# mrluin/TextualDegRemoval

Measured on AMD Instinct MI355X. Metric: train images/sec (512x512, bs=4/GPU), higher is better.
Workload: dtype f32 (3xbf16-split MFMA: 24-bit operand significands on the full fp32 exponent range, fp32 accumulate; unscaled gradients, no loss scale, no step-skip guard; tensors fp32 -- the MASA-encoder ResidualBlock activations / gradients as three bf16 planes whose sum IS the fp32 value, bit for bit)

## Files before the change

### textualdegremoval_amd/csrc/tdr_masa.hip

```cpp
#include "tdr_common.h"
#include "../../include/tdr.h"

namespace {

__device__ __forceinline__ int wrap_idx(int v, int n) { return v < 0 ? v + n : v; }

__global__ void lr_blocks_fwd_kernel(const float* __restrict__ feat, int C, int H, int W, int py, int px, int ky, int kx,
                                     long total, float* __restrict__ blk) {
    const int BH = ky + 2, BW = kx + 2;
    for (long i = blockIdx.x * (long)blockDim.x + threadIdx.x; i < total; i += (long)gridDim.x * blockDim.x) {
        const int u = (int)(i % BW); long r = i / BW;
        const int v = (int)(r % BH); r /= BH;
        const int c = (int)(r % C); r /= C;
        const int p = (int)(r % (py * px)); const long n = r / (py * px);
        const int by = p / px, bx = p % px;
        const int y = min(max(by * ky + v - 1, 0), H - 1), x = min(max(bx * kx + u - 1, 0), W - 1);
        blk[i] = feat[((n * C + c) * H + y) * W + x];
    }
}

__global__ void lr_blocks_bwd_kernel(const float* __restrict__ dblk, int C, int H, int W, int py, int px, int ky, int kx,
                                     long total, float* __restrict__ dfeat) {
    const int BH = ky + 2, BW = kx + 2, P = py * px;
    for (long i = blockIdx.x * (long)blockDim.x + threadIdx.x; i < total; i += (long)gridDim.x * blockDim.x) {
        const int x = (int)(i % W); long r = i / W;
        const int y = (int)(r % H); r /= H;
        const int c = (int)(r % C); const long n = r / C;
        float s = 0.f;
        for (int Y = (y == 0 ? 0 : y + 1); Y <= (y == H - 1 ? H + 1 : y + 1); ++Y) {
            for (int X = (x == 0 ? 0 : x + 1); X <= (x == W - 1 ? W + 1 : x + 1); ++X) {
                for (int by = max(0, (Y - 2) / ky - 1); by < py && by * ky <= Y; ++by) {
                    const int v = Y - by * ky;
                    if (v < 0 || v >= BH) continue;
                    for (int bx = max(0, (X - 2) / kx - 1); bx < px && bx * kx <= X; ++bx) {
                        const int u = X - bx * kx;
                        if (u < 0 || u >= BW) continue;
                        s += dblk[(((n * P + by * px + bx) * C + c) * BH + v) * BW + u];
                    }
                }
            }
        }
        dfeat[i] = s;
    }
}

__global__ __launch_bounds__(1024) void patch_inv_norm_kernel(const float* __restrict__ x, int C, int H, int W, int OH,
                                                             int OW, int dil, int step, int off, long npos,
                                                             float* __restrict__ inv) {
    __shared__ float red[16][64];
    const int lane = threadIdx.x & 63, sl = threadIdx.x >> 6;
    const long pos = blockIdx.x * 64L + lane;
    const bool live = pos < npos;
    const long pc = live ? pos : npos - 1;
    const int ox = (int)(pc % OW); const long r = pc / OW;
    const int oy = (int)(r % OH); const long b = r / OH;
    int offs[9];
#pragma unroll
    for (int k = 0; k < 9; ++k) {
        const int yy = oy * step + off + (k / 3) * dil, xx = ox * step + off + (k % 3) * dil;
        offs[k] = (yy >= 0 && yy < H && xx >= 0 && xx < W) ? yy * W + xx : -1;
    }
    float s = 0.f;
    const long HW = (long)H * W;
    for (int c = sl; c < C; c += 16) {
        const float* xc = x + (b * C + c) * HW;
#pragma unroll
        for (int k = 0; k < 9; ++k) {
            const float v = offs[k] >= 0 ? xc[offs[k]] : 0.f;
            s += v * v;
        }
    }
    red[sl][lane] = s;
    __syncthreads();
    if (sl == 0 && live) {
        float t = 0.f;
#pragma unroll
        for (int q = 0; q < 16; ++q) t += red[q][lane];
        inv[pos] = 1.0f / fmaxf(sqrtf(t), 1e-12f);
    }
}

__global__ __launch_bounds__(256) void patch_inv_norm_wave_kernel(const float* __restrict__ x, int C, int H, int W, int OH,
                                                                 int OW, int dil, int step, int off, long npos,
                                                                 float* __restrict__ inv) {
    const long pos = blockIdx.x * 4L + (threadIdx.x >> 6);
    if (pos >= npos) return;
    const int lane = threadIdx.x & 63;
    const int ox = (int)(pos % OW); long r = pos / OW;
    const int oy = (int)(r % OH); const long b = r / OH;
    float s = 0.f;
    for (int c = lane; c < C; c += 64) {
        const float* xc = x + (b * C + c) * (long)H * W;
#pragma unroll
        for (int k = 0; k < 9; ++k) {
            const int yy = oy * step + off + (k / 3) * dil, xx = ox * step + off + (k % 3) * dil;
            if (yy >= 0 && yy < H && xx >= 0 && xx < W) {
                const float v = xc[(long)yy * W + xx];
                s += v * v;
            }
        }
    }
    s = wave_sum(s);
    if (lane == 0) inv[pos] = 1.0f / fmaxf(sqrtf(s), 1e-12f);
}

__device__ __forceinline__ int box_start(int idx, int size, int diameter) {
    int lo = idx - diameter / 2 - 1, hi = idx + diameter / 2 + 1;
    if (lo < 0) { lo = 0; hi = diameter + 1; }
    if (hi > size - 1) { hi = size - 1; lo = hi - (diameter + 1); }
    return lo;
}

__global__ __launch_bounds__(256) void coarse_argmax_box_kernel(const float* __restrict__ dots,
                                                               const float* __restrict__ invq,
                                                               const float* __restrict__ invk, int ND, int N, int P,
                                                               int Hr, int Wr, int diameter, int* __restrict__ index,
                                                               int* __restrict__ y1, int* __restrict__ x1) {
    __shared__ float sv[256];
    __shared__ int si[256];
    const int np = blockIdx.x, n = np / P;
    const int R = Hr * Wr;
    float best = -INFINITY; int bi = 0x7fffffff;
    for (int r = threadIdx.x; r < R; r += 256) {
        float s = 0.f;
        for (int d = 0; d < ND; ++d)
            s += dots[((long)d * N * P + np) * R + r] * invq[(long)d * N * P + np] * invk[((long)d * N + n) * R + r];
        if (s > best) { best = s; bi = r; }
    }
    sv[threadIdx.x] = best; si[threadIdx.x] = bi;
    __syncthreads();
    for (int o = 128; o > 0; o >>= 1) {
        if (threadIdx.x < o) {
            const float v2 = sv[threadIdx.x + o]; const int i2 = si[threadIdx.x + o];
            if (v2 > sv[threadIdx.x] || (v2 == sv[threadIdx.x] && i2 < si[threadIdx.x])) { sv[threadIdx.x] = v2; si[threadIdx.x] = i2; }
        }
        __syncthreads();
    }
    if (threadIdx.x == 0) {
        const int idx = si[0];
        index[np] = idx;
        x1[np] = box_start(idx % Wr, Wr, diameter);
        y1[np] = box_start(idx / Wr, Hr, diameter);
    }
}

__global__ void gather_ref_block_kernel(const float* __restrict__ feat, int C, int H, int W, const int* __restrict__ y1,
                                        const int* __restrict__ x1, int P, int side, int s, long total,
                                        float* __restrict__ out) {
    const int SS = side * s;
    for (long i = blockIdx.x * (long)blockDim.x + threadIdx.x; i < total; i += (long)gridDim.x * blockDim.x) {
        const int u = (int)(i % SS); long r = i / SS;
        const int v = (int)(r % SS); r /= SS;
        const int c = (int)(r % C); const long b = r / C;
        const long n = b / P;
        const int y = wrap_idx(y1[b] * s + v, H), x = wrap_idx(x1[b] * s + u, W);
        out[i] = feat[((n * C + c) * H + y) * W + x];
    }
}

__global__ void scatter_ref_block_kernel(const float* __restrict__ dblk, int C, int H, int W, const int* __restrict__ y1,
                                         const int* __restrict__ x1, int P, int side, long total,
                                         float* __restrict__ dfeat) {
    for (long i = blockIdx.x * (long)blockDim.x + threadIdx.x; i < total; i += (long)gridDim.x * blockDim.x) {
        const int x = (int)(i % W); long r = i / W;
        const int y = (int)(r % H); r /= H;
        const int c = (int)(r % C); const long n = r / C;
        float acc = 0.f;
        for (int p = 0; p < P; ++p) {
            const long b = n * P + p;
            const int by = y1[b], bx = x1[b];
#pragma unroll
            for (int wy = 0; wy < 2; ++wy) {
                const int v = y - wy * H - by;
                if (v < 0 || v >= side || (wy == 1) != (by + v < 0)) continue;
#pragma unroll
                for (int wx = 0; wx < 2; ++wx) {
                    const int u = x - wx * W - bx;
                    if (u < 0 || u >= side || (wx == 1) != (bx + u < 0)) continue;
                    acc += dblk[((b * C + c) * side + v) * side + u];
                }
            }
        }
        dfeat[i] += acc;
    }
}

__global__ __launch_bounds__(256) void fine_argmax_kernel(const float* __restrict__ dots, const float* __restrict__ invq,
                                                         const float* __restrict__ invk, long rows, int P, int R,
                                                         int* __restrict__ index_all, float* __restrict__ soft_att) {
    const long row = blockIdx.x * 4L + (threadIdx.x >> 6);
    if (row >= rows) return;
    const int lane = threadIdx.x & 63;
    const long b = row / P;
    const float iq = invq[row];
    float best = -INFINITY; int bi = 0x7fffffff;
    for (int r = lane; r < R; r += 64) {
        const float v = dots[row * R + r] * iq * invk[b * R + r];
        if (v > best) { best = v; bi = r; }
    }
#pragma unroll
    for (int o = 32; o > 0; o >>= 1) {
        const float v2 = __shfl_xor(best, o, 64); const int i2 = __shfl_xor(bi, o, 64);
        if (v2 > best || (v2 == best && i2 < bi)) { best = v2; bi = i2; }
    }
    if (lane == 0) { index_all[row] = bi; soft_att[row] = best; }
}

__global__ __launch_bounds__(256) void fine_search_bwd_kernel(const float* __restrict__ datt,
                                                             const float* __restrict__ soft_att,
                                                             const int* __restrict__ index_all,
                                                             const float* __restrict__ lrb, const float* __restrict__ refb,
                                                             const float* __restrict__ invq, const float* __restrict__ invk,
                                                             int C, int K, int D, float* __restrict__ dlrb,
                                                             float* __restrict__ drefb) {
    extern __shared__ float sm[];
    const int b = blockIdx.y, c = blockIdx.x;
    const int P = K * K, BS = K + 2, R1 = D - 2;
    float* s_da = sm;
    float* s_at = s_da + P;
    float* s_iq = s_at + P;
    float* s_ik = s_iq + P;
    int* s_ix = reinterpret_cast<int*>(s_ik + P);
    float* s_q = reinterpret_cast<float*>(s_ix + P);
    float* s_k = s_q + BS * BS;
    int* s_ry = reinterpret_cast<int*>(s_k + D * D);
    int* s_rx = s_ry + P;
    int* s_qo = s_rx + P;
    for (int p = threadIdx.x; p < P; p += 256) {
        const int ix = index_all[(long)b * P + p];
        s_da[p] = datt[(long)b * P + p];
        s_at[p] = soft_att[(long)b * P + p];
        s_iq[p] = invq[(long)b * P + p];
        s_ik[p] = invk[(long)b * R1 * R1 + ix];
        s_ix[p] = ix;
        s_ry[p] = ix / R1;
        s_rx[p] = ix % R1;
        s_qo[p] = (p / K) * BS + (p % K);
    }
    for (int i = threadIdx.x; i < BS * BS; i += 256) s_q[i] = lrb[((long)b * C + c) * BS * BS + i];
    for (int i = threadIdx.x; i < D * D; i += 256) s_k[i] = refb[((long)b * C + c) * D * D + i];
    __syncthreads();
    for (int i = threadIdx.x; i < BS * BS; i += 256) {
        const int y = i / BS, x = i % BS;
        float s = 0.f;
#pragma unroll
        for (int k = 0; k < 9; ++k) {
            const int pyy = y - k / 3, pxx = x - k % 3;
            if (pyy < 0 || pyy >= K || pxx < 0 || pxx >= K) continue;
            const int p = pyy * K + pxx;
            const int ry = s_ry[p], rx = s_rx[p];
            const float kv = s_k[(ry + k / 3) * D + rx + k % 3];
            s += s_da[p] * s_iq[p] * (kv * s_ik[p] - s_at[p] * s_q[i] * s_iq[p]);
        }
        dlrb[((long)b * C + c) * BS * BS + i] = s;
    }
    for (int i = threadIdx.x; i < D * D; i += 256) {
        const int v = i / D, u = i % D;
        float s = 0.f;
        for (int p = 0; p < P; ++p) {
            const int kyy = v - s_ry[p], kxx = u - s_rx[p];
            if (kyy < 0 || kyy > 2 || kxx < 0 || kxx > 2) continue;
            const float qv = s_q[s_qo[p] + kyy * BS + kxx];
            s += s_da[p] * s_ik[p] * (qv * s_iq[p] - s_at[p] * s_k[i] * s_ik[p]);
        }
        drefb[((long)b * C + c) * D * D + i] = s;
    }
}

struct TrGeom {
    int src[9];
    float wgt;
    float inv_cnt;
    int a00, a01, a10, a11; float w00, w01, w10, w11;
};

__device__ __forceinline__ void tr_geometry(int Yl, int Xl, int b, const int* __restrict__ y1, const int* __restrict__ x1,
                                            const int* __restrict__ index_all, const float* __restrict__ soft_att, int K,
                                            int side, int s, int H, int W, TrGeom& g) {
    const int R1 = side - 2;
    const int i0 = Yl / s, j0 = Xl / s;
    int cnt = 0;
#pragma unroll
    for (int k = 0; k < 9; ++k) {
        const int i = i0 + k / 3 - 1, j = j0 + k % 3 - 1;
        g.src[k] = -1;
        if (i < 0 || i >= K || j < 0 || j >= K) continue;
        const int idx = index_all[(long)b * K * K + i * K + j];
        const int ry = idx / R1, rx = idx % R1;
        const int sy = ry * s + Yl - i * s + s, sx = rx * s + Xl - j * s + s;
        const int gy = wrap_idx(y1[b] * s + sy, H), gx = wrap_idx(x1[b] * s + sx, W);
        g.src[k] = gy * W + gx;
        ++cnt;
    }
    g.inv_cnt = 1.0f / (float)cnt;
    const float fy = fmaxf(((float)Yl + 0.5f) / (float)s - 0.5f, 0.f), fx = fmaxf(((float)Xl + 0.5f) / (float)s - 0.5f, 0.f);
    const int yy0 = min((int)fy, K - 1), xx0 = min((int)fx, K - 1);
    const int yy1 = min(yy0 + 1, K - 1), xx1 = min(xx0 + 1, K - 1);
    const float ly = fy - (float)yy0, lx = fx - (float)xx0;
    g.a00 = yy0 * K + xx0; g.a01 = yy0 * K + xx1; g.a10 = yy1 * K + xx0; g.a11 = yy1 * K + xx1;
    g.w00 = (1.f - ly) * (1.f - lx); g.w01 = (1.f - ly) * lx; g.w10 = ly * (1.f - lx); g.w11 = ly * lx;
    const float* at = soft_att + (long)b * K * K;
    const float top = at[g.a00] * (1.f - lx) + at[g.a01] * lx;
    const float bot = at[g.a10] * (1.f - lx) + at[g.a11] * lx;
    g.wgt = (top * (1.f - ly) + bot * ly);
}

constexpr int TR_CG = 8;

__global__ __launch_bounds__(256) void transfer_fwd_kernel(const float* __restrict__ feat, int C, int H, int W,
                                                          const int* __restrict__ y1, const int* __restrict__ x1,
                                                          const int* __restrict__ index_all,
                                                          const float* __restrict__ soft_att, int py, int px, int K,
                                                          int side, int s, float* __restrict__ out, long out_ns) {
    const int OW = px * K * s, OH = py * K * s;
    const int pix = blockIdx.x * 256 + threadIdx.x, n = blockIdx.z;
    if (pix >= OH * OW) return;
    const int Y = pix / OW, X = pix % OW;
    const int by = Y / (K * s), bx = X / (K * s);
    const int b = (n * py + by) * px + bx;
    TrGeom g;
    tr_geometry(Y - by * K * s, X - bx * K * s, b, y1, x1, index_all, soft_att, K, side, s, H, W, g);
    const long HWf = (long)H * W, HWo = (long)OH * OW;
    float mult[9];
#pragma unroll
    for (int k = 0; k < 9; ++k) {
        int m = 0;
        bool first = g.src[k] >= 0;
#pragma unroll
        for (int q = 0; q < 9; ++q) {
            const bool same = g.src[q] == g.src[k];
            m += same ? 1 : 0;
            if (q < k && same) first = false;
        }
        mult[k] = first ? (float)m : 0.f;
    }
    const int c0 = blockIdx.y * TR_CG;
    float accs[TR_CG];
#pragma unroll
    for (int i = 0; i < TR_CG; ++i) {
        const float* f = feat + ((long)n * C + min(c0 + i, C - 1)) * HWf;
        float acc = 0.f;
#pragma unroll
        for (int k = 0; k < 9; ++k)
            if (mult[k] != 0.f) acc += mult[k] * f[g.src[k]];
        accs[i] = acc;
    }
#pragma unroll
    for (int i = 0; i < TR_CG; ++i)
        if (c0 + i < C) out[(long)n * out_ns + (long)(c0 + i) * HWo + pix] = accs[i] * g.inv_cnt * g.wgt;
}

__global__ __launch_bounds__(256) void absmax_bits_kernel(const float* __restrict__ x, long x_ns, long per4, int N,
                                                         unsigned* __restrict__ out) {
    float m = 0.f;
    const f32x4* p = reinterpret_cast<const f32x4*>(x + (long)blockIdx.y * x_ns);
    for (long i = blockIdx.x * 256L + threadIdx.x; i < per4; i += (long)gridDim.x * 256) {
        const f32x4 v = p[i];
        m = fmaxf(fmaxf(m, fmaxf(fabsf(v[0]), fabsf(v[1]))), fmaxf(fabsf(v[2]), fabsf(v[3])));
    }
    m = wave_max(m);
    if ((threadIdx.x & 63) == 0) atomicMax(out, __float_as_uint(m));
}
__device__ __forceinline__ int fixed_shift(unsigned amax_bits) {
    const int e = (int)((amax_bits >> 23) & 0xff) - 127;
    return 46 - (e + 1);
}
__global__ void fixed_to_float_kernel(const long long* __restrict__ acc, long n, const unsigned* __restrict__ amax_bits,
                                      float* __restrict__ out) {
    const double inv = ldexp(1.0, -fixed_shift(amax_bits[0]));
    for (long i = blockIdx.x * 256L + threadIdx.x; i < n; i += (long)gridDim.x * 256) out[i] += (float)((double)acc[i] * inv);
}

template <bool FIXED>
__global__ __launch_bounds__(256) void transfer_bwd_kernel(const float* __restrict__ dout, long dout_ns,
                                                          const float* __restrict__ feat, int C, int H, int W,
                                                          const int* __restrict__ y1, const int* __restrict__ x1,
                                                          const int* __restrict__ index_all,
                                                          const float* __restrict__ soft_att, int py, int px, int K,
                                                          int side, int s, int cpb , int N,
                                                          const unsigned* __restrict__ amax_bits,
                                                          unsigned long long* __restrict__ dfacc ,
                                                          float* __restrict__ dfeat ,
                                                          float* __restrict__ dA ) {
    const int OW = px * K * s, OH = py * K * s;
    const int pix = blockIdx.x * 256 + threadIdx.x, n = blockIdx.z;
    if (pix >= OH * OW) return;
    const int Y = pix / OW, X = pix % OW;
    const int by = Y / (K * s), bx = X / (K * s);
    const int b = (n * py + by) * px + bx;
    TrGeom g;
    tr_geometry(Y - by * K * s, X - bx * K * s, b, y1, x1, index_all, soft_att, K, side, s, H, W, g);
    const long HWf = (long)H * W, HWo = (long)OH * OW;
    const float coef = g.inv_cnt * g.wgt;
    float mult[9];
#pragma unroll
    for (int k = 0; k < 9; ++k) {
        int m = 0;
        bool first = g.src[k] >= 0;
#pragma unroll
        for (int q = 0; q < 9; ++q) {
            const bool same = g.src[q] == g.src[k];
            m += same ? 1 : 0;
            if (q < k && same) first = false;
        }
        mult[k] = first ? (float)m : 0.f;
    }
    float da = 0.f;
    const int c0 = blockIdx.y * cpb, c1 = min(c0 + cpb, C);
    const int shift = FIXED ? fixed_shift(amax_bits[0]) : 0;
    const bool scatter = !FIXED || amax_bits[0] != 0u;
    for (int c = c0; c < c1; ++c) {
        const float* f = feat + ((long)n * C + c) * HWf;
        const float go = dout[(long)n * dout_ns + (long)c * HWo + pix];
        float acc = 0.f;
        const float gv = go * coef;
#pragma unroll
        for (int k = 0; k < 9; ++k)
            if (mult[k] > 0.f) {
                acc += mult[k] * f[g.src[k]];
                if (!scatter) continue;
                if (FIXED) atomicAdd(&dfacc[((long)n * C + c) * HWf + g.src[k]], (unsigned long long)__float2ll_rn(ldexpf(gv * mult[k], shift)));
                else atomicAdd(&dfeat[((long)n * C + c) * HWf + g.src[k]], gv * mult[k]);
            }
        da += go * acc * g.inv_cnt;
    }
    dA[((long)blockIdx.y * N + n) * HWo + pix] = da;
}

__global__ __launch_bounds__(64) void transfer_datt_kernel(const float* __restrict__ dA, int py, int px, int K, int s,
                                                          int chunks, long chunk_stride, float* __restrict__ datt) {
    const int b = blockIdx.x, e = blockIdx.y;
    const int P = py * px, n = b / P, by = (b % P) / px, bx = b % px;
    const int i = e / K, j = e % K;
    const int OW = px * K * s, OH = py * K * s, KS = K * s;
    const int ylo = max((i - 1) * s, 0), yhi = min((i + 2) * s, KS);
    const int xlo = max((j - 1) * s, 0), xhi = min((j + 2) * s, KS);
    const int nw = xhi - xlo, tot = (yhi - ylo) * nw;
    float acc = 0.f;
    for (int t = threadIdx.x; t < tot; t += 64) {
        const int Yl = ylo + t / nw, Xl = xlo + t % nw;
        const float fy = fmaxf(((float)Yl + 0.5f) / (float)s - 0.5f, 0.f), fx = fmaxf(((float)Xl + 0.5f) / (float)s - 0.5f, 0.f);
        const int yy0 = min((int)fy, K - 1), xx0 = min((int)fx, K - 1);
        const int yy1 = min(yy0 + 1, K - 1), xx1 = min(xx0 + 1, K - 1);
        const float ly = fy - (float)yy0, lx = fx - (float)xx0;
        float wgt = 0.f;
        if (yy0 == i && xx0 == j) wgt += (1.f - ly) * (1.f - lx);
        if (yy0 == i && xx1 == j) wgt += (1.f - ly) * lx;
        if (yy1 == i && xx0 == j) wgt += ly * (1.f - lx);
        if (yy1 == i && xx1 == j) wgt += ly * lx;
        if (wgt != 0.f) {
            const long o = (long)n * OH * OW + (long)(by * KS + Yl) * OW + bx * KS + Xl;
            float v = 0.f;
            for (int q = 0; q < chunks; ++q) v += dA[q * chunk_stride + o];
            acc += wgt * v;
        }
    }
    acc = wave_sum(acc);
    if (threadIdx.x == 0) datt[(long)b * K * K + e] += acc;
}

inline int grid1d(long total, int cap = 8192) {
    long b = (total + 255) / 256;
    return (int)(b < cap ? (b < 1 ? 1 : b) : cap);
}

}

extern "C" int tdr_lr_blocks_fwd(const float* feat, int N, int C, int H, int W, int py, int px, int ky, int kx, float* blk,
                                 void* stream) {
    TDR_REQUIRE(feat && blk, "tdr_lr_blocks_fwd: null pointer");
    const long total = (long)N * py * px * C * (ky + 2) * (kx + 2);
    hipLaunchKernelGGL(lr_blocks_fwd_kernel, dim3(grid1d(total)), dim3(256), 0, (hipStream_t)stream, feat, C, H, W, py, px, ky,
                       kx, total, blk);
    TDR_LAUNCH_CHECK("lr_blocks_fwd");
    return TDR_OK;
}

extern "C" int tdr_lr_blocks_bwd(const float* dblk, int N, int C, int H, int W, int py, int px, int ky, int kx,
                                 float* dfeat, void* stream) {
    TDR_REQUIRE(dblk && dfeat, "tdr_lr_blocks_bwd: null pointer");
    const long total = (long)N * C * H * W;
    hipLaunchKernelGGL(lr_blocks_bwd_kernel, dim3(grid1d(total)), dim3(256), 0, (hipStream_t)stream, dblk, C, H, W, py, px, ky,
                       kx, total, dfeat);
    TDR_LAUNCH_CHECK("lr_blocks_bwd");
    return TDR_OK;
}

extern "C" int tdr_patch_inv_norm(const float* x, int B, int C, int H, int W, int OH, int OW, int dil, int pad, int step,
                                  int off, float* inv, void* stream) {
    TDR_REQUIRE(x && inv, "tdr_patch_inv_norm: null pointer");
    const long npos = (long)B * OH * OW;
    if (npos >= 1024)
        hipLaunchKernelGGL(patch_inv_norm_kernel, dim3((unsigned)((npos + 63) / 64)), dim3(1024), 0, (hipStream_t)stream, x, C, H,
                           W, OH, OW, dil, step, off - pad, npos, inv);
    else
        hipLaunchKernelGGL(patch_inv_norm_wave_kernel, dim3((unsigned)((npos + 3) / 4)), dim3(256), 0, (hipStream_t)stream, x, C,
                           H, W, OH, OW, dil, step, off - pad, npos, inv);
    TDR_LAUNCH_CHECK("patch_inv_norm");
    return TDR_OK;
}

extern "C" int tdr_coarse_argmax_box(const float* dots, const float* invq, const float* invk, int ND, int N, int P, int Hr,
                                     int Wr, int diameter, int* index, int* y1, int* x1, void* stream) {
    TDR_REQUIRE(dots && invq && invk && index && y1 && x1, "tdr_coarse_argmax_box: null pointer");
    hipLaunchKernelGGL(coarse_argmax_box_kernel, dim3(N * P), dim3(256), 0, (hipStream_t)stream, dots, invq, invk, ND, N, P, Hr,
                       Wr, diameter, index, y1, x1);
    TDR_LAUNCH_CHECK("coarse_argmax_box");
    return TDR_OK;
}

extern "C" int tdr_gather_ref_block(const float* feat, int N, int C, int H, int W, const int* y1, const int* x1, int P,
                                    int side, int s, float* out, void* stream) {
    TDR_REQUIRE(feat && y1 && x1 && out, "tdr_gather_ref_block: null pointer");
    const long total = (long)N * P * C * side * s * side * s;
    hipLaunchKernelGGL(gather_ref_block_kernel, dim3(grid1d(total)), dim3(256), 0, (hipStream_t)stream, feat, C, H, W, y1, x1,
                       P, side, s, total, out);
    TDR_LAUNCH_CHECK("gather_ref_block");
    return TDR_OK;
}

extern "C" int tdr_scatter_ref_block(const float* dblk, int N, int C, int H, int W, const int* y1, const int* x1, int P,
                                     int side, float* dfeat, void* stream) {
    TDR_REQUIRE(dblk && y1 && x1 && dfeat, "tdr_scatter_ref_block: null pointer");
    const long total = (long)N * C * H * W;
    hipLaunchKernelGGL(scatter_ref_block_kernel, dim3(grid1d(total)), dim3(256), 0, (hipStream_t)stream, dblk, C, H, W, y1, x1,
                       P, side, total, dfeat);
    TDR_LAUNCH_CHECK("scatter_ref_block");
    return TDR_OK;
}

extern "C" int tdr_fine_argmax(const float* dots, const float* invq, const float* invk, int B, int P, int R, int* index_all,
                               float* soft_att, void* stream) {
    TDR_REQUIRE(dots && invq && invk && index_all && soft_att, "tdr_fine_argmax: null pointer");
    const long rows = (long)B * P;
    hipLaunchKernelGGL(fine_argmax_kernel, dim3((unsigned)((rows + 3) / 4)), dim3(256), 0, (hipStream_t)stream, dots, invq, invk,
                       rows, P, R, index_all, soft_att);
    TDR_LAUNCH_CHECK("fine_argmax");
    return TDR_OK;
}

extern "C" int tdr_fine_search_bwd(const float* datt, const float* soft_att, const int* index_all, const float* lrb,
                                   const float* refb, const float* invq, const float* invk, int B, int C, int K, int D,
                                   float* dlrb, float* drefb, void* stream) {
    TDR_REQUIRE(datt && soft_att && index_all && lrb && refb && invq && invk && dlrb && drefb, "tdr_fine_search_bwd: null pointer");
    const size_t lds = (size_t)(8 * K * K + (K + 2) * (K + 2) + D * D) * sizeof(float);
    hipLaunchKernelGGL(fine_search_bwd_kernel, dim3(C, B), dim3(256), lds, (hipStream_t)stream, datt, soft_att, index_all, lrb,
                       refb, invq, invk, C, K, D, dlrb, drefb);
    TDR_LAUNCH_CHECK("fine_search_bwd");
    return TDR_OK;
}

extern "C" int tdr_transfer_fwd(const float* feat, int N, int C, int H, int W, const int* y1, const int* x1,
                                const int* index_all, const float* soft_att, int py, int px, int K, int side, int s,
                                float* out, int64_t out_ns, void* stream) {
    TDR_REQUIRE(feat && y1 && x1 && index_all && soft_att && out, "tdr_transfer_fwd: null pointer");
    const long opix = (long)py * K * s * px * K * s;
    hipLaunchKernelGGL(transfer_fwd_kernel, dim3((unsigned)((opix + 255) / 256), tdr_cdiv(C, TR_CG), N), dim3(256), 0,
                       (hipStream_t)stream, feat, C, H, W, y1, x1, index_all, soft_att, py, px, K, side, s, out, (long)out_ns);
    TDR_LAUNCH_CHECK("transfer_fwd");
    return TDR_OK;
}

static int tdr_transfer_chunks(int N, int C, int py, int px, int K, int s) {
    const long opix = (long)py * K * s * px * K * s;
    const long pix_blocks = ((opix + 255) / 256) * N;
    long chunks = (1024 + pix_blocks - 1) / pix_blocks;
    if (chunks > C / 8) chunks = C / 8;
    if (chunks < 1) chunks = 1;
    return (int)chunks;
}

extern "C" int64_t tdr_transfer_ws_floats(int N, int C, int H, int W, int py, int px, int K, int s) {
    const int64_t opix = (int64_t)py * K * s * px * K * s;
    return (int64_t)tdr_transfer_chunks(N, C, py, px, K, s) * N * opix + 4 + 2 * (int64_t)N * C * H * W;
}

extern "C" int tdr_transfer_bwd(const float* dout, int64_t dout_ns, const float* feat, int N, int C, int H, int W,
                                const int* y1, const int* x1, const int* index_all, const float* soft_att, int py, int px,
                                int K, int side, int s, int deterministic, float* dfeat, float* datt, float* ws, void* stream) {
    TDR_REQUIRE(dout && feat && y1 && x1 && index_all && soft_att && dfeat && datt && ws, "tdr_transfer_bwd: null pointer");
    const long opix = (long)py * K * s * px * K * s;
    hipStream_t st = (hipStream_t)stream;
    const int chunks = tdr_transfer_chunks(N, C, py, px, K, s);
    const int cpb = tdr_cdiv(C, chunks);
    float* dA = ws;
    const dim3 grid((unsigned)((opix + 255) / 256), tdr_cdiv(C, cpb), N);
    if (!deterministic) {
        hipLaunchKernelGGL(transfer_bwd_kernel<false>, grid, dim3(256), 0, st, dout, (long)dout_ns, feat, C, H, W, y1, x1, index_all,
                           soft_att, py, px, K, side, s, cpb, N, (const unsigned*)nullptr, (unsigned long long*)nullptr, dfeat, dA);
    } else {
        TDR_REQUIRE(opix % 4 == 0 && dout_ns % 4 == 0 && (reinterpret_cast<uintptr_t>(dout) & 15) == 0, "tdr_transfer_bwd: dout must be 16-byte aligned");
        char* tail = reinterpret_cast<char*>(ws + (long)chunks * N * opix);
        tail += (8 - reinterpret_cast<uintptr_t>(tail) % 8) % 8;
        unsigned* amax = reinterpret_cast<unsigned*>(tail);
        unsigned long long* acc = reinterpret_cast<unsigned long long*>(tail + 8);
        const long nacc = (long)N * C * H * W;
        if (hipMemsetAsync(tail, 0, 8 + (size_t)nacc * 8, st) != hipSuccess) {
            tdr_set_error("tdr_transfer_bwd: hipMemsetAsync failed");
            return TDR_ERR_HIP;
        }
        const long per4 = (long)C * opix / 4;
        hipLaunchKernelGGL(absmax_bits_kernel, dim3(grid1d(per4, 512), N), dim3(256), 0, st, dout, (long)dout_ns, per4, N, amax);
        hipLaunchKernelGGL(transfer_bwd_kernel<true>, grid, dim3(256), 0, st, dout, (long)dout_ns, feat, C, H, W, y1, x1, index_all,
                           soft_att, py, px, K, side, s, cpb, N, amax, acc, (float*)nullptr, dA);
        hipLaunchKernelGGL(fixed_to_float_kernel, dim3(grid1d(nacc, 4096)), dim3(256), 0, st, reinterpret_cast<const long long*>(acc),
                           nacc, amax, dfeat);
    }
    hipLaunchKernelGGL(transfer_datt_kernel, dim3(N * py * px, K * K), dim3(64), 0, st, ws, py, px, K, s, tdr_cdiv(C, cpb),
                       (long)N * opix, datt);
    TDR_LAUNCH_CHECK("transfer_bwd");
    return TDR_OK;
}

__global__ __launch_bounds__(256) void absmax_bits_any_kernel(const float* __restrict__ x, long x_ns, long per, unsigned* __restrict__ slot) {
    const float* p = x + (long)blockIdx.y * x_ns;
    float m = 0.f;
    unsigned bad = 0;
    for (long i = blockIdx.x * 256L + threadIdx.x; i < per; i += (long)gridDim.x * 256) {
        const float v = fabsf(p[i]);
        if (!(v <= 3.4028235e38f)) bad = 0x7fc00000u;
        m = fmaxf(m, v);
    }
    unsigned b = __float_as_uint(m) | bad;
#pragma unroll
    for (int o = 32; o > 0; o >>= 1) b = max(b, (unsigned)__shfl_xor((int)b, o, 64));
    if ((threadIdx.x & 63) == 0) atomicMax(slot, b);
}

extern "C" int tdr_absmax_bits(const float* x, int64_t x_ns, int N, int64_t per, unsigned* slot, void* stream) {
    TDR_REQUIRE(x && slot && N > 0 && per > 0, "tdr_absmax_bits: bad argument");
    hipLaunchKernelGGL(absmax_bits_any_kernel, dim3(grid1d(per, 256), N), dim3(256), 0, (hipStream_t)stream, x, (long)x_ns, (long)per, slot);
    TDR_LAUNCH_CHECK("absmax_bits");
    return TDR_OK;
}
```

Measured before the change: 62.79.

## Batch channels per block in MASA backward kernels and unroll datt gather

fine_search_bwd now handles eight channels per block and reuses the per-patch geometry and attention scalars across them. transfer_bwd processes channels in groups of eight, so all loads for a group are issued before the scatter atomics, using 32-bit byte offsets and a launch-bounds occupancy hint. transfer_datt unrolls its chunk-sum gather four ways. These target the latency-bound MASA backward kernels. The costs are more LDS and registers per block, and fewer blocks for fine_search.

```diff
diff --git a/profiles/masa_bwd/ab_kernels.py b/profiles/masa_bwd/ab_kernels.py
--- /dev/null
+++ b/profiles/masa_bwd/ab_kernels.py
@@ -0,0 +1,158 @@
+import argparse
+import hashlib
+import json
+import os
+import shutil
+import subprocess
+import sys
+import tempfile
+
+ROOT = os.path.dirname(os.path.dirname(os.path.dirname(os.path.abspath(__file__))))
+N, PY, PX, KK, SIDE, HD = 4, 4, 4, 8, 15, 32
+LEVELS = [(16, 32), (8, 64), (4, 128), (2, 256), (1, 512)]
+PATTERNS = ('coherent', 'random')
+FINE = (64, 512, 8, 15)
+
+
+def digest(t):
+    return hashlib.sha256(t.detach().cpu().contiguous().numpy().tobytes()).hexdigest()[:16]
+
+
+def index_pattern(kind, B, K, R1, g):
+    import torch
+    if kind == 'random':
+        return torch.randint(0, R1 * R1, (B, K * K), generator=g)
+    r0 = torch.randint(0, R1 - K + 1, (B, 1, 1), generator=g)
+    c0 = torch.randint(0, R1 - K + 1, (B, 1, 1), generator=g)
+    return ((r0 + torch.arange(K).view(1, K, 1)) * R1 + c0 + torch.arange(K).view(1, 1, K)).reshape(B, K * K)
+
+
+def transfer_inputs(s, C, pattern):
+    import torch
+    g = torch.Generator().manual_seed(1000 * s + C + (7 if pattern == 'random' else 0))
+    B = N * PY * PX
+    return dict(feat=torch.randn(N, C, HD * s, HD * s, generator=g).cuda(),
+                dout=torch.randn(N, C, PY * KK * s, PX * KK * s, generator=g).cuda(),
+                y1=torch.randint(0, HD - SIDE + 1, (B,), generator=g).int().cuda(),
+                x1=torch.randint(0, HD - SIDE + 1, (B,), generator=g).int().cuda(),
+                index_all=index_pattern(pattern, B, KK, SIDE - 2, g).int().cuda(),
+                soft_att=(torch.rand(B, KK * KK, generator=g) * 0.8 + 0.2).cuda())
+
+
+def graph_time(fn):
+    import torch
+    fn()
+    torch.cuda.synchronize()
+    st = torch.cuda.Stream()
+    with torch.cuda.stream(st):
+        fn()
+        gr = torch.cuda.CUDAGraph()
+        with torch.cuda.graph(gr, stream=st):
+            for _ in range(20):
+                fn()
+    torch.cuda.synchronize()
+    gr.replay()
+    torch.cuda.synchronize()
+    ts = []
+    for _ in range(15):
+        a, b = torch.cuda.Event(enable_timing=True), torch.cuda.Event(enable_timing=True)
+        a.record()
+        gr.replay()
+        b.record()
+        torch.cuda.synchronize()
+        ts.append(a.elapsed_time(b) * 1000.0 / 20)
+    return sorted(ts)[len(ts) // 2]
+
+
+def child(tag, folder):
+    import torch
+    sys.path.insert(0, ROOT)
+    from textualdegremoval_amd import kernels as K
+    out = dict(lib=os.environ.get('TDR_LIB_PATH', 'default'), bits={}, us={})
+    for s, C in LEVELS:
+        for pattern in PATTERNS:
+            inp = transfer_inputs(s, C, pattern)
+            key = f's={s} C={C} {pattern}'
+
+            def run(det, dfeat, datt):
+                K.DETERMINISTIC = det
+                K.transfer_bwd(inp['dout'], inp['feat'], inp['y1'], inp['x1'], inp['index_all'], inp['soft_att'], PY, PX, KK, SIDE, s, dfeat, datt)
+
+            B = N * PY * PX
+            rec = {}
+            for det in (True, False):
+                for rep in range(1 if det else 2):
+                    dfeat, datt = torch.zeros_like(inp['feat']), torch.zeros(B, KK * KK, device='cuda')
+                    run(det, dfeat, datt)
+                    torch.cuda.synchronize()
+                    if det:
+                        rec['det dfeat'], rec['det datt'] = digest(dfeat), digest(datt)
+                    else:
+                        rec['float datt'] = digest(datt)
+                        if tag == 'parent' or rep == 0:
+                            torch.save(dfeat.cpu(), os.path.join(folder, f'{tag} {key} float{rep}.pt'))
+            out['bits'][key] = rec
+            dfeat, datt = torch.zeros_like(inp['feat']), torch.zeros(B, KK * KK, device='cuda')
+            for det in (False, True):
+                out['us'][f'{key} {"fixed" if det else "float"}'] = graph_time(lambda: run(det, dfeat, datt))
+            del inp, dfeat, datt
+    B, C, Kk, D = FINE
+    for pattern in PATTERNS:
+        g = torch.Generator().manual_seed(99 + (7 if pattern == 'random' else 0))
+        lrb, refb = torch.randn(B, C, Kk + 2, Kk + 2, generator=g).cuda(), torch.randn(B, C, D, D, generator=g).cuda()
+        datt, att = torch.randn(B, Kk * Kk, generator=g).cuda(), torch.rand(B, Kk * Kk, generator=g).cuda()
+        invq, invk = (torch.rand(B, Kk * Kk, generator=g) + 0.5).cuda(), (torch.rand(B, (D - 2) ** 2, generator=g) + 0.5).cuda()
+        ia = index_pattern(pattern, B, Kk, D - 2, g).int().cuda()
+        dl, dr = K.fine_search_bwd(datt, att, ia, lrb, refb, invq, invk, Kk, D)
+        torch.cuda.synchronize()
+        key = f'fine B={B} C={C} {pattern}'
+        out['bits'][key] = {'dlrb': digest(dl), 'drefb': digest(dr)}
+        out['us'][key] = graph_time(lambda: K.fine_search_bwd(datt, att, ia, lrb, refb, invq, invk, Kk, D))
+    with open(os.path.join(folder, tag + '.json'), 'w') as f:
+        json.dump(out, f)
+
+
+def main():
+    ap = argparse.ArgumentParser()
+    ap.add_argument('--parent')
+    ap.add_argument('--result', default=os.path.join(ROOT, 'textualdegremoval_amd', 'libtdr_hip.so'))
+    ap.add_argument('--child')
+    ap.add_argument('--dir')
+    a = ap.parse_args()
+    if a.child:
+        return child(a.child, a.dir)
+    import torch
+    folder = tempfile.mkdtemp(prefix='masa_bwd_ab_')
+    try:
+        for tag, lib in (('parent', a.parent), ('result', a.result)):
+            env = dict(os.environ, TDR_LIB_PATH=os.path.abspath(lib))
+            subprocess.run([sys.executable, os.path.abspath(__file__), '--child', tag, '--dir', folder], env=env, check=True, timeout=400)
+        P, R = (json.load(open(os.path.join(folder, t + '.json'))) for t in ('parent', 'result'))
+        print(f'parent {P["lib"]}\nresult {R["lib"]}\n')
+        print('## Bit identity, parent library against result (sha256 of the tensor bytes)\n')
+        print('| case | output | parent | result | |\n|---|---|---|---|---|')
+        bad = 0
+        for key, rec in P['bits'].items():
+            for name, h in rec.items():
+                same = R['bits'][key][name] == h
+                bad += not same
+                print(f'| {key} | {name} | {h} | {R["bits"][key][name]} | {"equal" if same else "DIFFERENT"} |')
+        print(f'\n{bad} outputs differ.\n')
+        print('## Float-atomic dfeat: max |a - b| / max |a|, two runs of the parent beside parent against result\n')
+        print('| case | max abs dfeat | parent run 0 vs run 1 | parent run 0 vs result run 0 |\n|---|---|---|---|')
+        for s, C in LEVELS:
+            for pattern in PATTERNS:
+                key = f's={s} C={C} {pattern}'
+                p0, p1, r0 = (torch.load(os.path.join(folder, f'{t} {key} float{i}.pt')).double() for t, i in (('parent', 0), ('parent', 1), ('result', 0)))
+                m = p0.abs().max().item()
+                print(f'| {key} | {m:.3e} | {(p0 - p1).abs().max().item() / m:.3e} | {(p0 - r0).abs().max().item() / m:.3e} |')
+        print('\n## Time per launch, microseconds (graph of 20, median of 15 replays)\n')
+        print('| launch | parent | result | result / parent |\n|---|---|---|---|')
+        for key, t in P['us'].items():
+            print(f'| {key} | {t:.1f} | {R["us"][key]:.1f} | {R["us"][key] / t:.2f} |')
+    finally:
+        shutil.rmtree(folder, ignore_errors=True)
+
+
+if __name__ == '__main__':
+    main()
diff --git a/profiles/masa_bwd/masa_rows.py b/profiles/masa_bwd/masa_rows.py
--- /dev/null
+++ b/profiles/masa_bwd/masa_rows.py
@@ -0,0 +1,58 @@
+import bisect
+import re
+import sqlite3
+import sys
+
+MASA = ('transfer_bwd_kernel', 'fine_search_bwd_kernel', 'transfer_datt_kernel')
+
+
+def short(n):
+    n = re.sub(r'\(anonymous namespace\)::', '', n)
+    return re.sub(r'\(.*', '', re.sub(r'^void ', '', n))
+
+
+def main():
+    c = sqlite3.connect(sys.argv[1])
+    rows = list(c.execute('select name, start, end, grid_x/workgroup_x, grid_y, grid_z, vgpr_count, lds_size from kernels '
+                          'where name not like "%spin_kernel%" order by start'))
+    steps = sum('fine_search_bwd_kernel' in r[0] for r in rows)
+    tot = sum(r[2] - r[1] for r in rows)
+    print(f'total kernel time {tot / 1e6 / steps:.2f} ms/step over {steps} steps; {len(rows) / steps:.0f} launches/step')
+    ev = sorted([(r[1], 1) for r in rows] + [(r[2], -1) for r in rows])
+    t, n, run = [], [], 0
+    for at, d in ev:
+        run += d
+        t.append(at)
+        n.append(run)
+    busy = sum(t[i + 1] - t[i] for i in range(len(t) - 1) if n[i] >= 1)
+    both = sum(t[i + 1] - t[i] for i in range(len(t) - 1) if n[i] >= 2)
+    print(f'some kernel running {busy / 1e6 / steps:.2f} ms/step, two or more running {both / 1e6 / steps:.2f} ms/step')
+
+    def shared(a, b):
+        s, i = 0, bisect.bisect_right(t, a) - 1
+        while i < len(t) - 1 and t[i] < b:
+            if n[i] >= 2:
+                s += min(t[i + 1], b) - max(t[i], a)
+            i += 1
+        return s
+
+    by_name, by_grid = {}, {}
+    for name, a, b, gx, gy, gz, vg, lds in rows:
+        k = short(name)
+        if not any(m in k for m in MASA):
+            continue
+        for d, key in ((by_name, k), (by_grid, (k, gx, gy, gz, vg, lds))):
+            e = d.setdefault(key, [0, 0, 0])
+            e[0] += 1
+            e[1] += b - a
+            e[2] += shared(a, b)
+    print('--- MASA backward kernels (the last column: share of their time with another kernel running)')
+    for k, (cnt, dur, sh) in sorted(by_name.items(), key=lambda x: -x[1][1]):
+        print(f'{dur / 1e6 / steps:8.3f} ms/step  n/step {cnt / steps:4.1f}  {k:32s} {100 * sh / dur:5.1f} %')
+    print('--- by grid (workgroups x,y,z)')
+    for (k, gx, gy, gz, vg, lds), (cnt, dur, sh) in sorted(by_grid.items(), key=lambda x: (x[0][0], -x[0][1])):
+        print(f'{dur / cnt / 1e3:8.1f} us  n/step {cnt / steps:4.1f}  grid({gx},{gy},{gz}) vgpr {vg} lds {lds}  {k:32s} {100 * sh / dur:5.1f} %')
+
+
+if __name__ == '__main__':
+    main()
diff --git a/textualdegremoval_amd/csrc/tdr_masa.hip b/textualdegremoval_amd/csrc/tdr_masa.hip
--- a/textualdegremoval_amd/csrc/tdr_masa.hip
+++ b/textualdegremoval_amd/csrc/tdr_masa.hip
@@ -206,6 +206,8 @@
     if (lane == 0) { index_all[row] = bi; soft_att[row] = best; }
 }
 
+constexpr int FS_FC = 8;
+
 __global__ __launch_bounds__(256) void fine_search_bwd_kernel(const float* __restrict__ datt,
                                                              const float* __restrict__ soft_att,
                                                              const int* __restrict__ index_all,
@@ -214,16 +216,16 @@
                                                              int C, int K, int D, float* __restrict__ dlrb,
                                                              float* __restrict__ drefb) {
     extern __shared__ float sm[];
-    const int b = blockIdx.y, c = blockIdx.x;
-    const int P = K * K, BS = K + 2, R1 = D - 2;
+    const int b = blockIdx.y, cg = blockIdx.x * FS_FC, nc = min(FS_FC, C - cg);
+    const int P = K * K, BS = K + 2, R1 = D - 2, BB = BS * BS, DD = D * D;
     float* s_da = sm;
     float* s_at = s_da + P;
     float* s_iq = s_at + P;
     float* s_ik = s_iq + P;
     int* s_ix = reinterpret_cast<int*>(s_ik + P);
     float* s_q = reinterpret_cast<float*>(s_ix + P);
-    float* s_k = s_q + BS * BS;
-    int* s_ry = reinterpret_cast<int*>(s_k + D * D);
+    float* s_k = s_q + FS_FC * BB;
+    int* s_ry = reinterpret_cast<int*>(s_k + FS_FC * DD);
     int* s_rx = s_ry + P;
     int* s_qo = s_rx + P;
     for (int p = threadIdx.x; p < P; p += 256) {
@@ -237,33 +239,50 @@
         s_rx[p] = ix % R1;
         s_qo[p] = (p / K) * BS + (p % K);
     }
-    for (int i = threadIdx.x; i < BS * BS; i += 256) s_q[i] = lrb[((long)b * C + c) * BS * BS + i];
-    for (int i = threadIdx.x; i < D * D; i += 256) s_k[i] = refb[((long)b * C + c) * D * D + i];
+    for (int i = threadIdx.x; i < FS_FC * BB; i += 256) s_q[i] = i < nc * BB ? lrb[((long)b * C + cg) * BB + i] : 0.f;
+    for (int i = threadIdx.x; i < FS_FC * DD; i += 256) s_k[i] = i < nc * DD ? refb[((long)b * C + cg) * DD + i] : 0.f;
     __syncthreads();
-    for (int i = threadIdx.x; i < BS * BS; i += 256) {
+    for (int i = threadIdx.x; i < BB; i += 256) {
         const int y = i / BS, x = i % BS;
-        float s = 0.f;
+        float s[FS_FC];
+#pragma unroll
+        for (int j = 0; j < FS_FC; ++j) s[j] = 0.f;
 #pragma unroll
         for (int k = 0; k < 9; ++k) {
             const int pyy = y - k / 3, pxx = x - k % 3;
             if (pyy < 0 || pyy >= K || pxx < 0 || pxx >= K) continue;
             const int p = pyy * K + pxx;
-            const int ry = s_ry[p], rx = s_rx[p];
-            const float kv = s_k[(ry + k / 3) * D + rx + k % 3];
-            s += s_da[p] * s_iq[p] * (kv * s_ik[p] - s_at[p] * s_q[i] * s_iq[p]);
-        }
-        dlrb[((long)b * C + c) * BS * BS + i] = s;
-    }
-    for (int i = threadIdx.x; i < D * D; i += 256) {
+            const int ko = (s_ry[p] + k / 3) * D + s_rx[p] + k % 3;
+            const float da = s_da[p], at = s_at[p], iq = s_iq[p], ik = s_ik[p];
+#pragma unroll
+            for (int j = 0; j < FS_FC; ++j) {
+                const float kv = s_k[j * DD + ko];
+                s[j] += da * iq * (kv * ik - at * s_q[j * BB + i] * iq);
+            }
+        }
+#pragma unroll
+        for (int j = 0; j < FS_FC; ++j)
+            if (j < nc) dlrb[((long)b * C + cg + j) * BB + i] = s[j];
+    }
+    for (int i = threadIdx.x; i < DD; i += 256) {
         const int v = i / D, u = i % D;
-        float s = 0.f;
+        float s[FS_FC], kc[FS_FC];
+#pragma unroll
+        for (int j = 0; j < FS_FC; ++j) { s[j] = 0.f; kc[j] = s_k[j * DD + i]; }
         for (int p = 0; p < P; ++p) {
             const int kyy = v - s_ry[p], kxx = u - s_rx[p];
             if (kyy < 0 || kyy > 2 || kxx < 0 || kxx > 2) continue;
-            const float qv = s_q[s_qo[p] + kyy * BS + kxx];
-            s += s_da[p] * s_ik[p] * (qv * s_iq[p] - s_at[p] * s_k[i] * s_ik[p]);
-        }
-        drefb[((long)b * C + c) * D * D + i] = s;
+            const int qo = s_qo[p] + kyy * BS + kxx;
+            const float da = s_da[p], at = s_at[p], iq = s_iq[p], ik = s_ik[p];
+#pragma unroll
+            for (int j = 0; j < FS_FC; ++j) {
+                const float qv = s_q[j * BB + qo];
+                s[j] += da * ik * (qv * iq - at * kc[j] * ik);
+            }
+        }
+#pragma unroll
+        for (int j = 0; j < FS_FC; ++j)
+            if (j < nc) drefb[((long)b * C + cg + j) * DD + i] = s[j];
     }
 }
 
@@ -371,17 +390,71 @@
     for (long i = blockIdx.x * 256L + threadIdx.x; i < n; i += (long)gridDim.x * 256) out[i] += (float)((double)acc[i] * inv);
 }
 
+#ifndef TDR_TRB_CG
+#define TDR_TRB_CG 8
+#endif
+constexpr int TRB_CG = TDR_TRB_CG;
+
+template <bool FIXED, bool FULL>
+__device__ __forceinline__ void transfer_bwd_group(const float* __restrict__ dout_n , unsigned& po , long HWo,
+                                                   const float* __restrict__ feat, long HWf, long nC, int cb, int nv,
+                                                   unsigned (&so)[9] , const float (&mult)[9], float coef, float inv_cnt,
+                                                   bool scatter, int shift, unsigned long long* __restrict__ dfacc,
+                                                   float* __restrict__ dfeat, float& da) {
+    const char* fp = reinterpret_cast<const char*>(feat + (nC + cb) * HWf);
+    const char* op = reinterpret_cast<const char*>(dout_n + (long)cb * HWo);
+    char* dp = FIXED ? reinterpret_cast<char*>(dfacc + (nC + cb) * HWf) : reinterpret_cast<char*>(dfeat + (nC + cb) * HWf);
+    asm volatile("" : "+v"(po));
+    float go[TRB_CG], fv[TRB_CG][9];
+#pragma unroll
+    for (int k = 0; k < 9; ++k) asm volatile("" : "+v"(so[k]));
+#pragma unroll
+    for (int i = 0; i < TRB_CG; ++i) {
+        const int j = FULL ? i : min(i, nv - 1);
+        go[i] = *reinterpret_cast<const float*>(op + j * HWo * 4 + po);
+    }
+#pragma unroll
+    for (int k = 0; k < 9; ++k)
+        if (mult[k] > 0.f) {
+#pragma unroll
+            for (int i = 0; i < TRB_CG; ++i) {
+                const int j = FULL ? i : min(i, nv - 1);
+                fv[i][k] = *reinterpret_cast<const float*>(fp + j * HWf * 4 + so[k]);
+            }
+        }
+#pragma unroll
+    for (int i = 0; i < TRB_CG; ++i) {
+        float acc = 0.f;
+#pragma unroll
+        for (int k = 0; k < 9; ++k)
+            if (mult[k] > 0.f) acc += mult[k] * fv[i][k];
+        if (FULL || i < nv) da += go[i] * acc * inv_cnt;
+    }
+    if (!scatter) return;
+#pragma unroll
+    for (int k = 0; k < 9; ++k)
+        if (mult[k] > 0.f) {
+#pragma unroll
+            for (int i = 0; i < TRB_CG; ++i) {
+                if (!FULL && i >= nv) continue;
+                const float gv = go[i] * coef;
+                if (FIXED) atomicAdd(reinterpret_cast<unsigned long long*>(dp + i * HWf * 8 + so[k] * 2u), (unsigned long long)__float2ll_rn(ldexpf(gv * mult[k], shift)));
+                else atomicAdd(reinterpret_cast<float*>(dp + i * HWf * 4 + so[k]), gv * mult[k]);
+            }
+        }
+}
+
 template <bool FIXED>
-__global__ __launch_bounds__(256) void transfer_bwd_kernel(const float* __restrict__ dout, long dout_ns,
-                                                          const float* __restrict__ feat, int C, int H, int W,
-                                                          const int* __restrict__ y1, const int* __restrict__ x1,
-                                                          const int* __restrict__ index_all,
-                                                          const float* __restrict__ soft_att, int py, int px, int K,
-                                                          int side, int s, int cpb , int N,
-                                                          const unsigned* __restrict__ amax_bits,
-                                                          unsigned long long* __restrict__ dfacc ,
-                                                          float* __restrict__ dfeat ,
-                                                          float* __restrict__ dA ) {
+__global__ __launch_bounds__(256, 4) void transfer_bwd_kernel(const float* __restrict__ dout, long dout_ns,
+                                                             const float* __restrict__ feat, int C, int H, int W,
+                                                             const int* __restrict__ y1, const int* __restrict__ x1,
+                                                             const int* __restrict__ index_all,
+                                                             const float* __restrict__ soft_att, int py, int px, int K,
+                                                             int side, int s, int cpb , int N,
+                                                             const unsigned* __restrict__ amax_bits,
+                                                             unsigned long long* __restrict__ dfacc ,
+                                                             float* __restrict__ dfeat ,
+                                                             float* __restrict__ dA ) {
     const int OW = px * K * s, OH = py * K * s;
     const int pix = blockIdx.x * 256 + threadIdx.x, n = blockIdx.z;
     if (pix >= OH * OW) return;
@@ -409,23 +482,21 @@
     const int c0 = blockIdx.y * cpb, c1 = min(c0 + cpb, C);
     const int shift = FIXED ? fixed_shift(amax_bits[0]) : 0;
     const bool scatter = !FIXED || amax_bits[0] != 0u;
-    for (int c = c0; c < c1; ++c) {
-        const float* f = feat + ((long)n * C + c) * HWf;
-        const float go = dout[(long)n * dout_ns + (long)c * HWo + pix];
-        float acc = 0.f;
-        const float gv = go * coef;
-#pragma unroll
-        for (int k = 0; k < 9; ++k)
-            if (mult[k] > 0.f) {
-                acc += mult[k] * f[g.src[k]];
-                if (!scatter) continue;
-                if (FIXED) atomicAdd(&dfacc[((long)n * C + c) * HWf + g.src[k]], (unsigned long long)__float2ll_rn(ldexpf(gv * mult[k], shift)));
-                else atomicAdd(&dfeat[((long)n * C + c) * HWf + g.src[k]], gv * mult[k]);
-            }
-        da += go * acc * g.inv_cnt;
-    }
+    const float* dout_n = dout + (long)n * dout_ns;
+    unsigned po = (unsigned)pix * 4u, so[9];
+#pragma unroll
+    for (int k = 0; k < 9; ++k) so[k] = (unsigned)g.src[k] * 4u;
+    int cb = c0;
+    for (; cb + TRB_CG <= c1; cb += TRB_CG)
+        transfer_bwd_group<FIXED, true>(dout_n, po, HWo, feat, HWf, (long)n * C, cb, TRB_CG, so, mult, coef, g.inv_cnt, scatter, shift,
+                                        dfacc, dfeat, da);
+    if (cb < c1)
+        transfer_bwd_group<FIXED, false>(dout_n, po, HWo, feat, HWf, (long)n * C, cb, c1 - cb, so, mult, coef, g.inv_cnt, scatter, shift,
+                                         dfacc, dfeat, da);
     dA[((long)blockIdx.y * N + n) * HWo + pix] = da;
 }
+
+constexpr int DATT_U = 4;
 
 __global__ __launch_bounds__(64) void transfer_datt_kernel(const float* __restrict__ dA, int py, int px, int K, int s,
                                                           int chunks, long chunk_stride, float* __restrict__ datt) {
@@ -437,23 +508,40 @@
     const int xlo = max((j - 1) * s, 0), xhi = min((j + 2) * s, KS);
     const int nw = xhi - xlo, tot = (yhi - ylo) * nw;
     float acc = 0.f;
-    for (int t = threadIdx.x; t < tot; t += 64) {
-        const int Yl = ylo + t / nw, Xl = xlo + t % nw;
-        const float fy = fmaxf(((float)Yl + 0.5f) / (float)s - 0.5f, 0.f), fx = fmaxf(((float)Xl + 0.5f) / (float)s - 0.5f, 0.f);
-        const int yy0 = min((int)fy, K - 1), xx0 = min((int)fx, K - 1);
-        const int yy1 = min(yy0 + 1, K - 1), xx1 = min(xx0 + 1, K - 1);
-        const float ly = fy - (float)yy0, lx = fx - (float)xx0;
-        float wgt = 0.f;
-        if (yy0 == i && xx0 == j) wgt += (1.f - ly) * (1.f - lx);
-        if (yy0 == i && xx1 == j) wgt += (1.f - ly) * lx;
-        if (yy1 == i && xx0 == j) wgt += ly * (1.f - lx);
-        if (yy1 == i && xx1 == j) wgt += ly * lx;
-        if (wgt != 0.f) {
-            const long o = (long)n * OH * OW + (long)(by * KS + Yl) * OW + bx * KS + Xl;
-            float v = 0.f;
-            for (int q = 0; q < chunks; ++q) v += dA[q * chunk_stride + o];
-            acc += wgt * v;
-        }
+    for (int t0 = threadIdx.x; t0 < tot; t0 += 64 * DATT_U) {
+        float w[DATT_U], v[DATT_U];
+        long o[DATT_U];
+#pragma unroll
+        for (int u = 0; u < DATT_U; ++u) {
+            const int t = t0 + 64 * u;
+            w[u] = 0.f; v[u] = 0.f; o[u] = 0;
+            if (t >= tot) continue;
+            const int Yl = ylo + t / nw, Xl = xlo + t % nw;
+            const float fy = fmaxf(((float)Yl + 0.5f) / (float)s - 0.5f, 0.f), fx = fmaxf(((float)Xl + 0.5f) / (float)s - 0.5f, 0.f);
+            const int yy0 = min((int)fy, K - 1), xx0 = min((int)fx, K - 1);
+            const int yy1 = min(yy0 + 1, K - 1), xx1 = min(xx0 + 1, K - 1);
+            const float ly = fy - (float)yy0, lx = fx - (float)xx0;
+            float wgt = 0.f;
+            if (yy0 == i && xx0 == j) wgt += (1.f - ly) * (1.f - lx);
+            if (yy0 == i && xx1 == j) wgt += (1.f - ly) * lx;
+            if (yy1 == i && xx0 == j) wgt += ly * (1.f - lx);
+            if (yy1 == i && xx1 == j) wgt += ly * lx;
+            w[u] = wgt;
+            o[u] = (long)n * OH * OW + (long)(by * KS + Yl) * OW + bx * KS + Xl;
+        }
+        for (int q = 0; q < chunks; ++q) {
+            float a[DATT_U];
+#pragma unroll
+            for (int u = 0; u < DATT_U; ++u) {
+                a[u] = 0.f;
+                if (w[u] != 0.f) a[u] = dA[q * chunk_stride + o[u]];
+            }
+#pragma unroll
+            for (int u = 0; u < DATT_U; ++u) v[u] += a[u];
+        }
+#pragma unroll
+        for (int u = 0; u < DATT_U; ++u)
+            if (w[u] != 0.f) acc += w[u] * v[u];
     }
     acc = wave_sum(acc);
     if (threadIdx.x == 0) datt[(long)b * K * K + e] += acc;
@@ -543,8 +631,9 @@
                                    const float* refb, const float* invq, const float* invk, int B, int C, int K, int D,
                                    float* dlrb, float* drefb, void* stream) {
     TDR_REQUIRE(datt && soft_att && index_all && lrb && refb && invq && invk && dlrb && drefb, "tdr_fine_search_bwd: null pointer");
-    const size_t lds = (size_t)(8 * K * K + (K + 2) * (K + 2) + D * D) * sizeof(float);
-    hipLaunchKernelGGL(fine_search_bwd_kernel, dim3(C, B), dim3(256), lds, (hipStream_t)stream, datt, soft_att, index_all, lrb,
+    const size_t lds = (size_t)(8 * K * K + FS_FC * ((K + 2) * (K + 2) + D * D)) * sizeof(float);
+    TDR_REQUIRE(B > 0 && C > 0 && lds <= 64 * 1024, "tdr_fine_search_bwd: the block does not fit the LDS");
+    hipLaunchKernelGGL(fine_search_bwd_kernel, dim3(tdr_cdiv(C, FS_FC), B), dim3(256), lds, (hipStream_t)stream, datt, soft_att, index_all, lrb,
                        refb, invq, invk, C, K, D, dlrb, drefb);
     TDR_LAUNCH_CHECK("fine_search_bwd");
     return TDR_OK;
@@ -580,6 +669,7 @@
                                 int K, int side, int s, int deterministic, float* dfeat, float* datt, float* ws, void* stream) {
     TDR_REQUIRE(dout && feat && y1 && x1 && index_all && soft_att && dfeat && datt && ws, "tdr_transfer_bwd: null pointer");
     const long opix = (long)py * K * s * px * K * s;
+    TDR_REQUIRE((long)H * W < (1L << 29) && opix < (1L << 30), "tdr_transfer_bwd: a channel plane is too large");
     hipStream_t st = (hipStream_t)stream;
     const int chunks = tdr_transfer_chunks(N, C, py, px, K, s);
     const int cpb = tdr_cdiv(C, chunks);
```

Measured after the change: 62.80, median of 2. No clear change (+0.0%).
